# joncampbell123/composite-video-simulator

Measured on AMD Instinct MI355X. Metric: frames/sec (output frames = fields; 720x486 NTSC, preset '-vhs'; steady-state pipelined throughput, 4 steps in flight), higher is better.
Workload: dtype f64; 1 GPU; 720x486 30fps 10s colour-bars clip, preset '-vhs': 300 frames -> 600 fields per GPU per step, frame-round-robin over 1 GPU(s); steps_in_flight=4, mode=exact (bit-identical to the reference: fp64, no FMA contraction)

## Files before the change

### composite-video-simulator_amd/csrc/ntsc_decode_fast.hip

```cpp
#pragma clang fp contract(off)

namespace ntscsim {
namespace fastdec {

typedef uint32_t v4u __attribute__((ext_vector_type(4)));
#ifdef NTSC_PLAIN_OUT_STORES
#define NTSC_OUT_STORE(p, v) (*(p) = (v))
#else
#define NTSC_OUT_STORE(p, v) __builtin_nontemporal_store((v), (p))
#endif
typedef __attribute__((address_space(1))) v4u *g_v4u_ptr;
typedef __attribute__((address_space(1))) const v4u *g_cv4u_ptr;
DEV v4u to_v4u(const uint4 &a) { return v4u{a.x, a.y, a.z, a.w}; }
typedef __attribute__((address_space(1))) uint32_t *g_u32_ptr;
typedef __attribute__((address_space(1))) const uint32_t *g_cu32_ptr;

#ifdef NTSC_NO_STEP_SCHED_BARRIER
#define NTSC_STEP_SCHED_BARRIER() ((void)0)
#else
#define NTSC_STEP_SCHED_BARRIER() __builtin_amdgcn_sched_barrier(0)
#endif

struct LaneRand32 {
    uint32_t p3, p2, p1;
    int pos;
    DEV void init(uint32_t *ring, const uint32_t *state, int stride, int lane, int o)
    {
        for (int j = 0; j < 31; j++) {
            const uint32_t w = state[(size_t)j * stride];
            const int sl = (o + j) & 31;
            ring[sl * 64 + lane] = w;
            if (sl == 0) ring[32 * 64 + lane] = w;
            if (j == 28) p3 = w;
            if (j == 29) p2 = w;
            if (j == 30) p1 = w;
        }
        pos = (o + 31) & 31;
    }
    DEV uint32_t next(uint32_t *ring, int lane)
    {
        const uint32_t v = ring[(pos + 1) * 64 + lane] + p3;
        ring[pos * 64 + lane] = v;
        if (pos == 0) ring[32 * 64 + lane] = v;
        p3 = p2; p2 = p1; p1 = v;
        pos = (pos + 1) & 31;
        return v >> 1;
    }
    template <int K>
    DEV uint32_t draw(uint32_t *rb, bool first_slot_is_zero)
    {
        const uint32_t v = rb[(K + 1) * 64] + p3;
        rb[K * 64] = v;
        if (K == 0 && first_slot_is_zero) rb[32 * 64] = v;
        p3 = p2; p2 = p1; p1 = v;
        return v >> 1;
    }
};

template <class RT>
struct Casc3;
template <>
struct Casc3<double> {
    double r0, r1, r2;
    DEV void reset(double v, double a) { const double r = v - (v * a); r0 = r1 = r2 = r; }
    DEV double push(double s, double a, double &m2)
    {
        const double p0 = (s * a) + r0;
        const double m0 = p0 * a;
        r0 = p0 - m0;
// ... 153 lines not shown
            if (ANY) {
                const int aL = odd ? o2 : e2, aH = odd ? o1 : e1;
                const int bL = odd ? e1 : o2, bH = odd ? ch : o1;
                a = hi ? aH : aL; b = hi ? bH : bL;
                const int sg = NEG ? ~mo : mo;
                a = (a ^ sg) - sg; b = (b ^ sg) - sg;
            } else {
                a = hi ? e1 : e2; b = hi ? o1 : o2;
                if (NEG) { a = -a; b = -b; }
            }
            e2 = e1; e1 = ch;
            if (MASK) { a &= dm; b &= dm; }
            ieN = a; qeN = b;
            Io = (ieP + ieN) >> 1;
            Qo = (qeP + qeN) >> 1;
        } else {
            o2 = o1; o1 = ch;
            Io = ieN; Qo = qeN;
            ieP = ieN; qeP = qeN;
        }
    }
};

template <bool VHS, class RT>
struct State {
    DemodR D1, D2;
    int l0, l1, l2, lsum;
    Casc3<RT> vl, vcU, vcV, sh, oU, oV;
    PoleHp<RT> vpre;
    int Yprev, Uraw, Vraw;
    RT Uf2[2];
    LaneRand32 rng;
    int nU, nV;
};

template <class RT, bool WR = false, bool BK = false, bool SV = false, bool XA = false, bool FO = false>
struct Const {
    static constexpr bool fullout = FO;
    static constexpr int SH = FO ? 3 : 0;
    RT a_oi, a_oq;
    uint32_t *xs;
    static constexpr bool wraps = WR;
    static constexpr bool back = BK;
    static constexpr bool svideo = SV;
    static constexpr bool anyxi = XA;
    bool odd;
    int mo;
    int ms[4];
    unsigned bmul, bshift;
    int wrapoff;
    int wrapA, wrapS;
    unsigned xi;
    bool hi;
    int W, xe, lane;
    int d, SKT, LOFF;
    int mL, mNL;
    int bA, bC;
    int dm;
    RT cosv, sinv;
    RT a_vc, a_vl, a_sh, a_tv, sharp2;
    int *tailU;
    size_t rstride;
    __amdgpu_buffer_rsrc_t comp;
    int vbase;
    int rowbytes;
};
// ... 94 lines not shown
{
    int Y, U, V;
    constexpr bool pick3 = ((J + 1 + CT::SH) & 1) != 0;
    constexpr bool neg3 = ((J + 1 + CT::SH) & 3) == 3;
    if constexpr (!VHS) {
        T.D1.template push<pick3, neg3, true, CT::back, true, CT::anyxi>(pc, C.hi, C.dm, Y, U, V, C.bmul, C.bshift, C.odd, C.mo);
    } else {
        int Yv, Uv, Vv;
        const int c2 = vcr_step<DPH, J, RT, CT>(P, S, T, C, pc, pl, Yv, Uv, Vv);
        if constexpr (CT::svideo) {
            Y = Yv; U = Uv & C.dm; V = Vv & C.dm;
        } else {
            T.D2.template push<pick3, neg3, true, false, true, CT::anyxi>(c2, C.hi, C.dm, Y, U, V, 0, 0, C.odd, C.mo);
        }
    }
    if constexpr (CT::fullout) {
        const int fUn = (int)S.oU.push((RT)U, C.a_oi);
        const RT fVd = rtrunc<RT>(S.oV.push((RT)V, C.a_oq));
        const int Yo = T.yd[J];
        T.yd[J] = Y;
        const RT fUd = (RT)T.ud[J & 1];
        T.ud[J & 1] = fUn;
        return yiq_to_bgra<RT>(Yo, fUd, fVd);
    } else {
        const RT fUd = rtrunc<RT>(S.oU.push((RT)U, C.a_tv));
        const RT fVd = rtrunc<RT>(S.oV.push((RT)V, C.a_tv));
        const int Yo = S.Yprev;
        S.Yprev = Y;
        return yiq_to_bgra<RT>(Yo, fUd, fVd);
    }
}

template <class RT, class CT>
DEV int vcr_edge(const DevParams &P, State<true, RT> &S, const CT &C, uint32_t *ring, int t, int &Yv, int &Uv, int &Vv)
{
    const int W = C.W;
    const int pc = t < W ? cs_load(C, t) : 0;
    int Y, U, V;
    S.D1.template push_edge<CT::back, CT::anyxi>(pc, t, C.xi, C.hi, W, C.xe, Y, U, V, C.bmul, C.bshift);
    const int x1 = t - 7;
    const bool in1 = x1 >= 0 && x1 < W;
    int fU = 0, fV = 0;
    if (in1) {
        U += S.nU; V += S.nV;
        S.nU = sdiv2(S.nU + (int)umod31(S.rng.next(ring, C.lane), P.m_cnoise) - P.cnoise_k);
        S.nV = sdiv2(S.nV + (int)umod31(S.rng.next(ring, C.lane), P.m_cnoise) - P.cnoise_k);
        const RT u = (RT)U, v = (RT)V;
        U = (int)((u * C.cosv) - (v * C.sinv));
        V = (int)((u * C.sinv) + (v * C.cosv));
        fU = (int)S.vcU.push((RT)U, C.a_vc);
        fV = (int)S.vcV.push((RT)V, C.a_vc);
        if (x1 >= W - C.d) {
            C.tailU[(size_t)(x1 & 15) * C.rstride] = U;
            C.tailU[(size_t)(16 + (x1 & 15)) * C.rstride] = V;
        }
    }
    const int x2 = x1 - C.d;
    const int xl = t - C.LOFF;
    const int pl = (xl >= 0 && xl < W) ? cs_load(C, xl) : 0;
    const int yb = sdiv4(S.l0 + S.l1 + S.l2 + pl);
    S.lsum = S.l1 + S.l2 + pl;
    S.l0 = S.l1; S.l1 = S.l2; S.l2 = pl;
    const bool in2 = x2 >= 0 && x2 < W;
    if (in2) {
        if (x2 >= W - C.d) {
            fU = C.tailU[(size_t)(x2 & 15) * C.rstride];
            fV = C.tailU[(size_t)(16 + (x2 & 15)) * C.rstride];
        }
        RT m2;
        RT s = S.vl.push((RT)yb, C.a_vl, m2);
        s += S.vpre.hp(s, m2, C.a_vl) * RT(1.6);
        const RT s0 = rtrunc<RT>(s);
        const RT ts = S.sh.push(s0, C.a_sh);
        Y = (int)(s0 + ((s0 - ts) * C.sharp2));
    }
    U = ((wave_up(fU) & C.bA) + fU + C.bC) >> C.bC;
    V = ((wave_up(fV) & C.bA) + fV + C.bC) >> C.bC;
    int c2 = 0;
    Yv = 0; Uv = 0; Vv = 0;
    if (in2) {
        Yv = Y; Uv = U; Vv = V;
        const unsigned s = (C.xi + (unsigned)x2) & 3u;
        int chroma = (s & 1u) ? V : U;
        if (s & 2u) chroma = -chroma;
        c2 = Y + chroma;
    }
    return c2;
}

template <bool VHS, class RT, class CT>
DEV bool edge_step(const DevParams &P, State<VHS, RT> &S, const CT &C, uint32_t *ring, int t,
                   uint32_t &px, int &xo_out)
{
    const int W = C.W;
    int Y, U, V;
    int x3 = t - 7;
    if constexpr (VHS) {
        int Yv, Uv, Vv;
        const int c2 = vcr_edge<RT, CT>(P, S, C, ring, t, Yv, Uv, Vv);
        const int x2 = t - 7 - C.d;
        if constexpr (CT::svideo) {
            Y = Yv; U = Uv; V = Vv;
            x3 = x2;
        } else {
            S.D2.template push_edge<false, CT::anyxi>(c2, x2, C.xi, C.hi, W, C.xe, Y, U, V);
            x3 = x2 - 7;
        }
    } else {
        const int pc = t < W ? cs_load(C, t) : 0;
        S.D1.template push_edge<CT::back, CT::anyxi>(pc, t, C.xi, C.hi, W, C.xe, Y, U, V, C.bmul, C.bshift);
    }
    if constexpr (CT::fullout) {
        if (x3 < 0 || x3 >= W + 4) return false;
        const bool in3f = x3 < W;
        if (!in3f) { U = 0; V = 0; Y = 0; }
        U &= C.dm; V &= C.dm;
        RT fUn = 0, fVn = 0;
        if (in3f) {
            fUn = rtrunc<RT>(S.oU.push((RT)U, C.a_oi));
            fVn = rtrunc<RT>(S.oV.push((RT)V, C.a_oq));
        }
        const int k3 = x3 & 3;
        const int Yo4 = (int)C.xs[k3 * 64], Ur4 = (int)C.xs[(4 + k3) * 64], Vr4 = (int)C.xs[(8 + k3) * 64];
        C.xs[k3 * 64] = (uint32_t)Y; C.xs[(4 + k3) * 64] = (uint32_t)U; C.xs[(8 + k3) * 64] = (uint32_t)V;
        const RT Uf = S.Uf2[0];
        S.Uf2[0] = S.Uf2[1]; S.Uf2[1] = fUn;
        const int xof = x3 - 4;
        if (xof < 0) return false;
        const RT Uo = xof < W - 2 ? Uf : (RT)Ur4;
        const RT Vo = xof < W - 4 ? fVn : (RT)Vr4;
        px = yiq_to_bgra<RT>(Yo4, Uo, Vo);
        xo_out = xof;
        return true;
    }
    if (x3 < 0 || x3 > W) return false;
    const bool in3 = x3 < W;
    if (!in3) { U = 0; V = 0; Y = 0; }
    U &= C.dm; V &= C.dm;
    RT fUd = 0, fVd = 0;
    if (in3) {
        fUd = rtrunc<RT>(S.oU.push((RT)U, C.a_tv));
        fVd = rtrunc<RT>(S.oV.push((RT)V, C.a_tv));
    }
    const int xo = x3 - 1;
    const int Yo = S.Yprev;
    const int Ur = S.Uraw, Vr = S.Vraw;
    S.Yprev = Y; S.Uraw = U; S.Vraw = V;
    if (xo < 0) return false;
    if (xo >= W - 1) { fUd = (RT)Ur; fVd = (RT)Vr; }
    px = yiq_to_bgra<RT>(Yo, fUd, fVd);
    xo_out = xo;
    return true;
}

template <bool VHS, int DPH, class RT, class CT>
DEV int steady(const DevParams &P, State<VHS, RT> &S, const CT &C, uint32_t *ring, uint32_t *lring,
               uint32_t *ostage, const unsigned long long *orow, uint32_t *drow, bool is_out, int t)
{
    const int t_end = C.W - (C.d > 7 ? C.d - 7 : 0);
    const int SKT = C.SKT, LOFF = C.LOFF, lane = C.lane;
    if (t + 4 > t_end) return t;
    if (VHS && (S.rng.pos & 7)) return t;
    Steady T;
    constexpr bool pick3_next = ((1 + CT::SH) & 1) != 0;
    T.D1.from(S.D1, VHS ? (DPH & 1) != 0 : pick3_next);
    T.D2.from(S.D2, pick3_next);
    T.lc1 = S.l2; T.lpA = S.l2 + S.l1; T.lpB = S.l1 + S.l0;
    if constexpr (CT::fullout) {
#pragma unroll
        for (int q = 0; q < 4; q++) T.yd[q] = (int)C.xs[q * 64];
        T.ud[0] = (int)S.Uf2[0]; T.ud[1] = (int)S.Uf2[1];
    }
    DemodS &Dout = (VHS && !CT::svideo) ? T.D2 : T.D1;
    if (!(VHS && CT::svideo)) { Dout.ieP &= C.dm; Dout.qeP &= C.dm; Dout.ieN &= C.dm; Dout.qeN &= C.dm; }
    int sbase = VHS ? S.rng.pos : 0;
    constexpr int PD = 4;
    int pc[PD], pl[PD];
#pragma unroll
    for (int j = 0; j < PD; j++) { pc[j] = cs_load(C, t + j); pl[j] = VHS ? cs_load<NTSC_COMP_LOAD2_AUX>(C, t + j - LOFF) : 0; }
    constexpr bool PFTOP = !VHS;
    int pend_x = -1;
#ifdef NTSC_FAST_LANE_STORE
#define NTSC_FAST_FLUSH()                                                                         \
    if (pend_x >= 0) {                                                                            \
        if (is_out) {                                                                             \
// ... 66 lines not shown
#pragma unroll
        for (int q = 0; q < 4; q++) C.xs[q * 64] = (uint32_t)T.yd[q];
        S.Uf2[0] = (RT)T.ud[0]; S.Uf2[1] = (RT)T.ud[1];
    }
    S.Uraw = 0; S.Vraw = 0;
    S.l2 = T.lc1; S.l1 = T.lpA - T.lc1; S.l0 = T.lpB - S.l1; S.lsum = S.l0 + S.l1 + S.l2;
    if (VHS) S.rng.pos = sbase;
    return t;
}

}

#ifndef NTSC_FAST_WAVES
#define NTSC_FAST_WAVES 2
#endif
#ifndef NTSC_FAST_WAVES_F32
#define NTSC_FAST_WAVES_F32 2
#endif
template <class RT> struct FastWaves { static constexpr int n = NTSC_FAST_WAVES; };
template <> struct FastWaves<float> { static constexpr int n = NTSC_FAST_WAVES_F32; };
template <bool VHS, class RT, bool WR, bool BK, bool SV = false, bool XA = false, bool FO = false>
DEV void decode_fast_body(const DevParams &P, const GeomDev &G, const FieldDev *__restrict__ fields,
                          const int *__restrict__ comp, const uint32_t *__restrict__ rs_chroma,
                          const int *__restrict__ n0_u, const int *__restrict__ n0_v,
                          const int *__restrict__ hs_shift, const int *__restrict__ pn_noise,
                          const int *__restrict__ dropout, int *__restrict__ tails)
{
    using namespace fastdec;
    __shared__ uint32_t ring[33 * 64];
    __shared__ uint32_t lring[FO ? 12 * 64 : 64];
    __shared__ __attribute__((aligned(16))) uint32_t ostage[64 * 20];
    __shared__ unsigned long long orow[64];

    const int lane = threadIdx.x;
    const int gidx = blockIdx.x * 63 + lane - 1;
    const int rc = gidx < 0 ? 0 : (gidx < P.R ? gidx : P.R - 1);
    const int f = rc / P.Lslot, k = rc - f * P.Lslot;
    const FieldDev &fd = fields[f];
    const unsigned field = fd.field & 1u;
    const bool rowok = (int)(field + 2u * k) < P.H;
#ifdef NTSC_AB_NOSTORE
    const bool is_out = false;
#else
    const bool is_out = lane >= 1 && gidx < P.R && rowok;
#endif
    const unsigned y = rowok ? field + 2u * (unsigned)k : field;
    const int W = P.W;
    uint32_t *drow = reinterpret_cast<uint32_t *>(fd.dst + (size_t)fd.dst_ls * y);
    orow[lane] = is_out ? (unsigned long long)drow : 0ull;
    const size_t tcol = (size_t)blockIdx.x * 64 + lane;
    const size_t tstride = (size_t)gridDim.x * 64;

    typedef Const<RT, WR, BK, SV, XA, FO> CT;
    CT C;
    C.bmul = P.m_amp_back.mul; C.bshift = P.m_amp_back.shift;
    C.xi = scan_phase(P, y, fd.fieldno);
    C.hi = (C.xi & 2u) != 0;
    C.odd = (C.xi & 1u) != 0;
    if constexpr (XA) {
        C.mo = opaque_v(C.odd ? -1 : 0);
#pragma unroll
        for (int j = 0; j < 4; j++) C.ms[j] = opaque_v(((C.xi + (unsigned)j) & 2u) ? -1 : 0);
    }
    C.W = W;
    C.xe = (W & 1) ? W - 1 : W - 2;
    C.lane = lane;
    C.d = VHS ? P.cdelay : 0;
    C.SKT = (VHS ? (CT::svideo ? 8 : 15) + C.d : 8) + CT::SH;
    C.LOFF = 5 + C.d;
    C.mL = opaque_v(C.hi ? -1 : 0);
    C.mNL = opaque_v(~C.mL);
    const bool vb = VHS && P.vblend && P.ntsc;
    C.bA = opaque_v((vb && k >= 2) ? -1 : 0);
    C.bC = opaque_v((vb && k >= 1) ? 1 : 0);
    C.dm = opaque_v((P.loss && dropout[rc] != 0) ? 0 : -1);
    C.cosv = 1; C.sinv = 0;
    if (VHS) {
        int n = (rowok ? pn_noise[rc] : 0) + P.pnoise_k;
        n = n < 0 ? 0 : (n > 2 * P.pnoise_k ? 2 * P.pnoise_k : n);
        C.cosv = (RT)G.ptab[2 * n]; C.sinv = (RT)G.ptab[2 * n + 1];
    }
    C.a_vc = (RT)P.a_vc; C.a_vl = (RT)P.a_vl; C.a_sh = (RT)P.a_sh; C.a_tv = (RT)P.a_tv;
    C.a_oi = (RT)P.a_in_i; C.a_oq = (RT)P.a_in_q;
    C.sharp2 = (RT)(P.sharpen * 2);
    C.tailU = tails + tcol;
    C.rstride = tstride;
    C.rowbytes = P.Rpad * 4;
    const int hs = P.hs ? hs_shift[rc] : 0;
    C.vbase = (int)((unsigned)rc * 4u + (unsigned)hs * (unsigned)C.rowbytes);
    {
        const int tw = W + W / 10;
        C.wrapoff = (int)((unsigned)(hs > 0 ? -tw : tw) * (unsigned)C.rowbytes);
        C.wrapA = hs > 0 ? tw - hs - 1 : (hs < 0 ? -hs - 1 : 0x3FFFFFFF);
        C.wrapS = opaque_v(hs < 0 ? -1 : 0);
    }
    C.comp = __builtin_amdgcn_make_buffer_rsrc(const_cast<int *>(comp), 0,
                                               (int)((unsigned)W * (unsigned)C.rowbytes), 0x00020000);

    State<VHS, RT> S;
    S.D1.init(); S.D2.init();
    S.l0 = S.l1 = S.l2 = S.lsum = 0;
    S.vl.reset(16, C.a_vl); S.vpre.reset(16, C.a_vl); S.vcU.reset(0, C.a_vc); S.vcV.reset(0, C.a_vc);
    S.sh.reset(0, C.a_sh);
    if (CT::fullout) { S.oU.reset(0, C.a_oi); S.oV.reset(0, C.a_oq); }
    else { S.oU.reset(0, C.a_tv); S.oV.reset(0, C.a_tv); }
    S.Yprev = S.Uraw = S.Vraw = 0;
    C.xs = lring + lane;
    if (CT::fullout)
        for (int q = 0; q < 12; q++) C.xs[q * 64] = 0;
    S.Uf2[0] = S.Uf2[1] = 0;
    S.nU = S.nV = 0;
    if (VHS) {
        const int fill_draws = 2 * (C.SKT - 7);
        S.rng.init(ring, rs_chroma + rc, P.Rpad, lane, (-(31 + fill_draws)) & 7);
        S.nU = n0_u[rc]; S.nV = n0_v[rc];
    }

    const int SKT = C.SKT;
    const int total = W + SKT;
    int t = 0;
#ifdef NTSC_EDGE_UNROLL
#pragma unroll NTSC_EDGE_UNROLL
#endif
    for (; t < SKT && t < total; t++) {
        uint32_t px; int xo;
        (void)edge_step<VHS, RT, CT>(P, S, C, ring, t, px, xo);
    }
    if constexpr (!VHS) t = steady<VHS, 0, RT, CT>(P, S, C, ring, lring, ostage, orow, drow, is_out, t);
    else switch ((C.SKT - 7) & 3) {
        case 0: t = steady<VHS, 0, RT, CT>(P, S, C, ring, lring, ostage, orow, drow, is_out, t); break;
        case 1: t = steady<VHS, 1, RT, CT>(P, S, C, ring, lring, ostage, orow, drow, is_out, t); break;
        case 2: t = steady<VHS, 2, RT, CT>(P, S, C, ring, lring, ostage, orow, drow, is_out, t); break;
        default: t = steady<VHS, 3, RT, CT>(P, S, C, ring, lring, ostage, orow, drow, is_out, t); break;
    }
#ifdef NTSC_EDGE_UNROLL
#pragma unroll NTSC_EDGE_UNROLL
#endif
    for (; t < total; t++) {
        uint32_t px; int xo;
        if (!edge_step<VHS, RT, CT>(P, S, C, ring, t, px, xo)) continue;
        ostage[lane * 20 + (xo & 15)] = px;
        if ((xo & 15) == 15) {
            if (is_out) {
                const uint4 *sp = reinterpret_cast<const uint4 *>(&ostage[lane * 20]);
                g_v4u_ptr dp = (g_v4u_ptr)(drow + (xo - 15));
                const uint4 a = sp[0], b = sp[1], c4 = sp[2], d4 = sp[3];
                dp[0] = to_v4u(a); dp[1] = to_v4u(b); dp[2] = to_v4u(c4); dp[3] = to_v4u(d4);
            }
        } else if (xo == W - 1 && is_out) {
            const int xb = xo & ~15;
            for (int q = xb; q <= xo; q++) ((g_u32_ptr)drow)[q] = ostage[lane * 20 + (q - xb)];
        }
    }
}

template <bool VHS, class RT, bool WR = false>
__global__ __launch_bounds__(64, VHS ? FastWaves<RT>::n : 4) void k_decode_fast(DevParams P, GeomDev G,
                                                     const FieldDev *__restrict__ fields,
                                                     const int *__restrict__ comp,
                                                     const uint32_t *__restrict__ rs_chroma,
                                                     const int *__restrict__ n0_u,
                                                     const int *__restrict__ n0_v,
                                                     const int *__restrict__ hs_shift,
                                                     const int *__restrict__ pn_noise,
                                                     const int *__restrict__ dropout,
                                                     int *__restrict__ tails)
{
    decode_fast_body<VHS, RT, WR, false>(P, G, fields, comp, rs_chroma, n0_u, n0_v, hs_shift, pn_noise, dropout, tails);
}

template <bool VHS, class RT>
__global__ __launch_bounds__(64, VHS ? FastWaves<RT>::n : 4) void k_decode_fast_bk(DevParams P, GeomDev G,
                                                     const FieldDev *__restrict__ fields,
                                                     const int *__restrict__ comp,
                                                     const uint32_t *__restrict__ rs_chroma,
                                                     const int *__restrict__ n0_u,
                                                     const int *__restrict__ n0_v,
                                                     const int *__restrict__ hs_shift,
                                                     const int *__restrict__ pn_noise,
                                                     const int *__restrict__ dropout,
                                                     int *__restrict__ tails)
{
    decode_fast_body<VHS, RT, VHS, true>(P, G, fields, comp, rs_chroma, n0_u, n0_v, hs_shift, pn_noise, dropout, tails);
}

template <class RT>
// ... 82 lines not shown
    C.d = P.cdelay;
    C.SKT = 7 + C.d;
    C.LOFF = 5 + C.d;
    C.mL = opaque_v(C.hi ? -1 : 0);
    C.mNL = opaque_v(~C.mL);
    const bool vb = P.vblend && P.ntsc;
    C.bA = opaque_v((vb && k >= 2) ? -1 : 0);
    C.bC = opaque_v((vb && k >= 1) ? 1 : 0);
    C.dm = -1;
    {
        int n = (rowok ? pn_noise[rc] : 0) + P.pnoise_k;
        n = n < 0 ? 0 : (n > 2 * P.pnoise_k ? 2 * P.pnoise_k : n);
        C.cosv = (RT)G.ptab[2 * n]; C.sinv = (RT)G.ptab[2 * n + 1];
    }
    C.a_vc = (RT)P.a_vc; C.a_vl = (RT)P.a_vl; C.a_sh = (RT)P.a_sh; C.a_tv = (RT)P.a_tv;
    C.sharp2 = (RT)(P.sharpen * 2);
    C.tailU = tails + tcol;
    C.rstride = tstride;
    C.rowbytes = P.Rpad * 4;
    const int hs = P.hs ? hs_shift[rc] : 0;
    C.vbase = (int)((unsigned)rc * 4u + (unsigned)hs * (unsigned)C.rowbytes);
    C.comp = __builtin_amdgcn_make_buffer_rsrc(const_cast<int *>(comp), 0,
                                               (int)((unsigned)W * (unsigned)C.rowbytes), 0x00020000);
    const __amdgpu_buffer_rsrc_t out = __builtin_amdgcn_make_buffer_rsrc(comp_out, 0,
                                               (int)((unsigned)W * (unsigned)C.rowbytes), 0x00020000);
    const int vout = (is_out ? gidx : P.R + lane) * 4;

    State<true, RT> S;
    S.D1.init(); S.D2.init();
    S.l0 = S.l1 = S.l2 = S.lsum = 0;
    S.vl.reset(16, C.a_vl); S.vpre.reset(16, C.a_vl); S.vcU.reset(0, C.a_vc); S.vcV.reset(0, C.a_vc);
    S.sh.reset(0, C.a_sh); S.oU.reset(0, C.a_tv); S.oV.reset(0, C.a_tv);
    S.Yprev = S.Uraw = S.Vraw = 0;
    S.rng.init(ring, rs_chroma + rc, P.Rpad, lane, (-(31 + 2 * (C.SKT - 7))) & 7);
    S.nU = n0_u[rc]; S.nV = n0_v[rc];

    const int SK1 = C.SKT, LOFF = C.LOFF;
    const int total = W + SK1;
    const unsigned rb = (unsigned)C.rowbytes;
    int t = 0;
    int yv_, uv_, vv_;
    for (; t < SK1 && t < total; t++) (void)vcr_edge<RT, CT>(P, S, C, ring, t, yv_, uv_, vv_);
    {
        const int t_end = W - (C.d > 7 ? C.d - 7 : 0);
        if (t + 4 <= t_end && !(S.rng.pos & 7)) {
            Steady T;
            T.D1.from(S.D1, (C.d & 1) != 0);
            T.D2.from(S.D2, true);
            T.lc1 = S.l2; T.lpA = S.l2 + S.l1; T.lpB = S.l1 + S.l0;
            int sbase = S.rng.pos;
            int pc[4], pl[4];
#pragma unroll
            for (int j = 0; j < 4; j++) { pc[j] = cs_load(C, t + j); pl[j] = cs_load<NTSC_COMP_LOAD2_AUX>(C, t + j - LOFF); }
            unsigned soff = (unsigned)(t - SK1) * rb;
#define NTSC_VCR_STEP(DPV, J)                                                                     \
            {                                                                                     \
                const int c2 = vcr_step<DPV, J, RT, CT>(P, S, T, C, pc[J], pl[J], yv_, uv_, vv_); \
                pc[J] = cs_load(C, t + 4 + J);         \
                pl[J] = cs_load<NTSC_COMP_LOAD2_AUX>(C, t + 4 + J - LOFF);                                             \
                __builtin_amdgcn_raw_buffer_store_b32(c2, out, vout, (int)soff, 0);               \
                soff += rb;                                                                       \
                NTSC_STEP_SCHED_BARRIER();                                                        \
            }
#define NTSC_VCR_ITER(DPV)                                                                        \
            for (; t + 4 <= t_end; t += 4) {                                                      \
                T.rb = ring + sbase * 64 + lane; T.rb0 = sbase == 0; sbase = (sbase + 8) & 31;    \
                NTSC_VCR_STEP(DPV, 0) NTSC_VCR_STEP(DPV, 1) NTSC_VCR_STEP(DPV, 2) NTSC_VCR_STEP(DPV, 3)  \
            }
            switch (C.d & 3) {
                case 0: NTSC_VCR_ITER(0) break;
                case 1: NTSC_VCR_ITER(1) break;
                case 2: NTSC_VCR_ITER(2) break;
                default: NTSC_VCR_ITER(3) break;
            }
#undef NTSC_VCR_ITER
#undef NTSC_VCR_STEP
            T.D1.to(S.D1, (C.d & 1) != 0);
            S.l2 = T.lc1; S.l1 = T.lpA - T.lc1; S.l0 = T.lpB - S.l1; S.lsum = S.l0 + S.l1 + S.l2;
            S.rng.pos = sbase;
        }
    }
    for (; t < total; t++) {
        const int c2 = vcr_edge<RT, CT>(P, S, C, ring, t, yv_, uv_, vv_);
        const int x2 = t - SK1;
        if (x2 >= 0) __builtin_amdgcn_raw_buffer_store_b32(c2, out, vout, (int)((unsigned)x2 * rb), 0);
    }
}

}
```

### composite-video-simulator_amd/csrc/ntsc_encode_fast.hip

```cpp
#pragma clang fp contract(off)

#ifndef NTSC_COMP_STORE_AUX
#define NTSC_COMP_STORE_AUX 2
#endif
#ifdef NTSC_ENC_LOAD_NT
#define NTSC_ENC_LOAD(p) __builtin_nontemporal_load(p)
#else
#define NTSC_ENC_LOAD(p) (*(p))
#endif
namespace ntscsim {
namespace fastenc {

using fastdec::Casc3;
using fastdec::opaque_v;

template <class RT>
struct EState {
    Casc3<RT> lpI, lpQ;
    int Yd[4];
    int Ir[4], Qr[4];
    int fI[2];
    fastdec::LaneRand32 rng;
    int noise;
    OnePoleT<RT> pre;
// ... 144 lines not shown
#pragma unroll
        for (int i = 0; i < 4; i++) {
            const int from = 16 * i + (lane >> 2);
            const unsigned l2 = (unsigned)__shfl((int)lo, from), h2 = (unsigned)__shfl((int)hi, from);
            ptr[i] = (const uint8_t *)(((uintptr_t)h2 << 32) | l2) + 16 * (lane & 3);
        }
        wr = (lane >> 2) * 20 + (lane & 3) * 4;
        rd = lane * 20;
    }
    DEV void request(int t0, fastdec::v4u (&q)[4]) const
    {
#pragma unroll
        for (int i = 0; i < 4; i++) q[i] = NTSC_ENC_LOAD((fastdec::g_cv4u_ptr)(ptr[i] + 4 * (size_t)t0));
    }
    DEV void deliver(const fastdec::v4u (&q)[4], uint32_t (&px)[16]) const
    {
#pragma unroll
        for (int i = 0; i < 4; i++) *reinterpret_cast<uint4 *>(&tile[16 * 20 * i + wr]) = make_uint4(q[i].x, q[i].y, q[i].z, q[i].w);
#pragma unroll
        for (int i = 0; i < 4; i++) {
            const uint4 v = *reinterpret_cast<const uint4 *>(&tile[rd + 4 * i]);
            px[4 * i] = v.x; px[4 * i + 1] = v.y; px[4 * i + 2] = v.z; px[4 * i + 3] = v.w;
        }
    }
};

}

template <class RT, bool PRE, bool XA = false, int GH = 0>
DEV void encode_fast_body(const DevParams &P, const FieldDev *__restrict__ fields, const uint32_t *__restrict__ rs_luma,
                          const int *__restrict__ n0_luma, int *__restrict__ comp)
{
    using namespace fastenc;
    __shared__ uint32_t ring[33 * 64];
#ifndef NTSC_ENC_NOCOOP
    __shared__ __attribute__((aligned(16))) uint32_t ltile[64 * 20];
#endif
    __shared__ uint32_t gring[GH ? NTSC_GHOST_RING * 64 : 1];
    const int lane = threadIdx.x;
    const int rho = blockIdx.x * 64 + lane;
    const int rc = rho < P.R ? rho : P.R - 1;
    const int f = rc / P.Lslot, k = rc - f * P.Lslot;
    const FieldDev &fd = fields[f];
    const unsigned field = fd.field & 1u;
    const bool valid = rho < P.R && (int)(field + 2u * k) < P.H;
    const unsigned y = valid ? field + 2u * (unsigned)k : field;
    const unsigned opposite = (fd.flags & 1u) ? ((fd.flags & 2u) ? 1u : 0u) : 0u;
    unsigned sy = y + opposite;
    if (sy > (unsigned)P.H - 1u) sy = (unsigned)P.H - 1u;
    const uint8_t *srow = fd.src + (size_t)fd.src_ls * sy;
    const int W = P.W;

    EConst<RT> C;
    C.xi = scan_phase(P, y, fd.fieldno);
    C.W = W;
    C.lane = lane;
    C.mL = opaque_v((C.xi & 2u) ? -1 : 0);
    C.mNL = opaque_v(~C.mL);
    C.odd = (C.xi & 1u) != 0;
#pragma unroll
    for (int j = 0; j < 4; j++) C.ms[j] = fastdec::opaque_v(((C.xi + (unsigned)j) & 2u) ? -1 : 0);
    C.a_i = (RT)P.a_in_i; C.a_q = (RT)P.a_in_q;
    C.a_pre = (RT)P.a_pre; C.pre_gain = (RT)P.pre_gain;
    C.rowbytes = P.Rpad * 4;
    C.vcol = rho * 4;
    C.comp = __builtin_amdgcn_make_buffer_rsrc(comp, 0, (int)((unsigned)W * (unsigned)C.rowbytes), 0x00020000);

    EState<RT> S;
    S.rng.init(ring, rs_luma + rc, P.Rpad, lane, 1);
    S.noise = n0_luma[rc];
    S.lpI.reset(0, C.a_i); S.lpQ.reset(0, C.a_q);
    S.pre.p = 16;
#pragma unroll
    for (int q = 0; q < 4; q++) { S.Yd[q] = 0; S.Ir[q] = 0; S.Qr[q] = 0; }
    S.fI[0] = S.fI[1] = 0;
    GhostRing<GH> gh;
    gh.begin(P, gring, lane);

    int t = 0;
    for (; t < 4; t++) edge_step<RT, PRE, GH>(P, S, C, ring, reinterpret_cast<const uint32_t *>(srow), t, gh);
    if (t + 16 <= W) {
#ifndef NTSC_ENC_NOCOOP
        CoopLoader L;
        L.begin(srow, ltile, lane);
        uint32_t cur[16];
        fastdec::v4u nq[4];
        L.request(t, nq);
        L.deliver(nq, cur);
#else
        uint32_t cur[16], nxt[16];
        load_chunk(srow, t, cur);
#endif
        int Y0 = S.Yd[0], Y1 = S.Yd[1], Y2 = S.Yd[2], Y3 = S.Yd[3];
        int I0 = S.fI[0], I1 = S.fI[1];
        RT IdT[4], QdT[4];
        int sbase = S.rng.pos;
        for (; t + 16 <= W; t += 16) {
            const bool more = t + 32 <= W;
            uint32_t *const rb = ring + sbase * 64 + lane;
            const bool rb0 = sbase == 0;
            sbase = (sbase + 16) & 31;
#ifndef NTSC_ENC_NOCOOP
            if (more) L.request(t + 16, nq);
#else
            if (more) load_chunk(srow, t + 16, nxt);
#endif
            unsigned soff = (unsigned)(t - 4) * (unsigned)C.rowbytes;
            int Yn[16], F[16];
#define NTSC_ENC_STEP(J, YX, IX)                                                                  \
            {                                                                                     \
                RT dY, Id_, Qd_;                                                                  \
                rgb_to_yiq256<RT>(cur[J], dY, Id_, Qd_);                                          \
                Yn[J] = (int)dY;                                                                  \
// ... 6 lines not shown
            NTSC_ENC_STEP(1, Y1, I1)
            NTSC_ENC_STEP(2, Y2, F[0])
            NTSC_ENC_STEP(3, Y3, F[1])
            NTSC_ENC_STEP(4, Yn[0], F[2])
            NTSC_ENC_STEP(5, Yn[1], F[3])
            NTSC_ENC_STEP(6, Yn[2], F[4])
            NTSC_ENC_STEP(7, Yn[3], F[5])
            NTSC_ENC_STEP(8, Yn[4], F[6])
            NTSC_ENC_STEP(9, Yn[5], F[7])
            NTSC_ENC_STEP(10, Yn[6], F[8])
            NTSC_ENC_STEP(11, Yn[7], F[9])
            NTSC_ENC_STEP(12, Yn[8], F[10])
            NTSC_ENC_STEP(13, Yn[9], F[11])
            NTSC_ENC_STEP(14, Yn[10], F[12])
            NTSC_ENC_STEP(15, Yn[11], F[13])
#undef NTSC_ENC_STEP
            Y0 = Yn[12]; Y1 = Yn[13]; Y2 = Yn[14]; Y3 = Yn[15];
            I0 = F[14]; I1 = F[15];
#ifndef NTSC_ENC_NOCOOP
            if (more) L.deliver(nq, cur);
#else
            if (more) {
#pragma unroll
                for (int j = 0; j < 16; j++) cur[j] = nxt[j];
            }
#endif
        }
        S.rng.pos = sbase;
        S.Yd[0] = Y0; S.Yd[1] = Y1; S.Yd[2] = Y2; S.Yd[3] = Y3;
        S.fI[0] = I0; S.fI[1] = I1;
#pragma unroll
        for (int q = 0; q < 4; q++) { S.Ir[q] = (int)IdT[q]; S.Qr[q] = (int)QdT[q]; }
    }
    for (; t < W + 4; t++) edge_step<RT, PRE, GH>(P, S, C, ring, reinterpret_cast<const uint32_t *>(srow), t, gh);
}

template <class RT>
__global__ __launch_bounds__(64) void k_encode_fast(DevParams P, const FieldDev *__restrict__ fields,
                                                    const uint32_t *__restrict__ rs_luma,
                                                    const int *__restrict__ n0_luma,
                                                    int *__restrict__ comp)
{
    encode_fast_body<RT, false>(P, fields, rs_luma, n0_luma, comp);
}

template <class RT, int GT>
__global__ __launch_bounds__(64) void k_encode_fast_gh(DevParams P, const FieldDev *__restrict__ fields,
                                                       const uint32_t *__restrict__ rs_luma,
                                                       const int *__restrict__ n0_luma,
                                                       int *__restrict__ comp)
{
    encode_fast_body<RT, false, false, GT>(P, fields, rs_luma, n0_luma, comp);
}

template <class RT>
__global__ __launch_bounds__(64) void k_encode_fast_xi(DevParams P, const FieldDev *__restrict__ fields,
                                                       const uint32_t *__restrict__ rs_luma,
                                                       const int *__restrict__ n0_luma,
                                                       int *__restrict__ comp)
{
    encode_fast_body<RT, false, true>(P, fields, rs_luma, n0_luma, comp);
}

template <class RT>
__global__ __launch_bounds__(64) void k_encode_fast_pre(DevParams P, const FieldDev *__restrict__ fields,
                                                        const uint32_t *__restrict__ rs_luma,
                                                        const int *__restrict__ n0_luma,
// ... 7 lines not shown
```

### composite-video-simulator_amd/csrc/ntscsim_hip.hip

```cpp
#include <hip/hip_runtime.h>

#include <algorithm>
#include <cmath>
#include <cstdio>
#include <cstdlib>
#include <cstring>
#include <mutex>
#include <unistd.h>
#include <new>
#include <string>
#include <vector>

#include "ntscsim.h"
#include "ntsc_device.hpp"

#include "ntsc_kernels.hip"
#include "ntsc_decode_fast.hip"
#include "ntsc_encode_fast.hip"
#include "ntsc_pipe.hip"
#include "ntsc422_kernels.hip"
#include "ntsc422_fused.hip"
#include "ntsc_scale.hip"
#include "ntsc_float.hpp"
#include "ntsc_blend.hpp"
// ... 486 lines not shown
        c->ev_free.push_back(s);
        n++;
    }
    c->ev_live.clear();
    if (n_calls) *n_calls = n;
    return NTSCSIM_OK;
}

extern "C" int ntscsim_set_mode(ntscsim_ctx *c, int mode)
{
    if (!c || (mode != NTSCSIM_MODE_EXACT && mode != NTSCSIM_MODE_FAST32 && mode != NTSCSIM_MODE_FLOAT)) return NTSCSIM_E_ARG;
    c->mode = mode;
    return NTSCSIM_OK;
}

extern "C" void ntscsim_debug_force_generic(ntscsim_ctx *c, int on)
{
    if (c) c->force_generic = on != 0;
}

extern "C" void ntscsim_debug_no_fast_decode(ntscsim_ctx *c, int on)
{
    if (c) { c->no_fast_decode = (on & 1) != 0; c->split_vhs = (on & 2) != 0; c->no_stream422 = (on & 4) != 0; c->no_ghost_fuse = (on & 8) != 0; c->no_setup_merge = (on & 16) != 0; }
}

extern "C" int ntscsim_debug_last_kernels(const ntscsim_ctx *c, char *out, size_t cap)
{
    if (!c || !out || cap == 0) return NTSCSIM_E_ARG;
    const size_t n = std::min(cap - 1, c->kernels.size());
    std::memcpy(out, c->kernels.data(), n);
    out[n] = 0;
    return (int)c->kernels.size();
}

extern "C" void ntscsim_debug_set_warmup(ntscsim_ctx *c, int luma_draws, int chroma_draws)
{
    if (!c) return;
    c->warm_override[0] = luma_draws;
    c->warm_override[1] = chroma_draws & ~1;
    (void)hipSetDevice(c->device);
    (void)hipDeviceSynchronize();
    for (Geometry *e : c->geoms) e->valid = false;
}

#ifndef NTSC_SETUP_MERGE_MAX
#define NTSC_SETUP_MERGE_MAX 64
#endif
static void launch_setup_kernels(ntscsim_ctx *c, const DevParams &D, const GeomDev &G, const FieldDev *fields_dev, int n, hipStream_t st,
                                 bool note, bool launch)
{
    const bool fs = D.hs || D.pnoise_k || D.loss, rs = D.noise_k || D.cnoise_k;
    if (fs && rs && n <= NTSC_SETUP_MERGE_MAX && !c->no_setup_merge) {
        const int nfs = 3 * n, nrs = (D.R + 63) / 64;
        if (note) note_kernel(c, "k_field_row_setup");
        if (launch)
        hipLaunchKernelGGL(k_field_row_setup, dim3((unsigned)(nfs + 2 * nrs)), dim3(64), 0, st, D, G, fields_dev,
                           c->hs_shift.p, c->pn_noise.p, c->dropout.p, c->rs_luma.p, c->n0_luma.p, c->rs_chroma.p,
                           c->n0_u.p, c->n0_v.p, nfs, nrs);
        return;
    }
    if (fs) {
        if (note) note_kernel(c, "k_field_setup");
        if (launch)
        hipLaunchKernelGGL(k_field_setup, dim3((n + 63) / 64), dim3(64), 0, st, D, G, fields_dev,
                           c->hs_shift.p, c->pn_noise.p, c->dropout.p);
    }
// ... 1501 lines not shown
```

Measured before the change: 805,800 frames/s.

## Prefetch edge samples ahead in decode edge loops and hoist per-row loads

Moves the composite sample loads out of the per-step edge function and issues them four steps ahead in a new edge_run loop, masking out-of-range values afterwards. The tail chroma read is prefetched one step early into state registers, and per-row side inputs (dropout, phase noise, h-shift, initial noise, RNG ring) are loaded at kernel entry. The RNG init is unrolled into batched loads. This is meant to hide global-memory latency in the serial head and tail phases, at the cost of extra registers and clamped redundant loads. Optional cycle-stamp probes are added behind a compile flag.

```diff
diff --git a/composite-video-simulator_amd/csrc/ntsc_decode_fast.hip b/composite-video-simulator_amd/csrc/ntsc_decode_fast.hip
--- a/composite-video-simulator_amd/csrc/ntsc_decode_fast.hip
+++ b/composite-video-simulator_amd/csrc/ntsc_decode_fast.hip
@@ -1,6 +1,24 @@
 #pragma clang fp contract(off)
 
 namespace ntscsim {
+#ifdef NTSC_PHASE_STAMPS
+__device__ unsigned long long g_phase_cycles[2][8];
+#define NTSC_PHASE_STAMP(v) const unsigned long long v = (unsigned long long)__builtin_readcyclecounter()
+DEV void phase_add(int which, int lane, unsigned long long t0, unsigned long long t1, unsigned long long t2,
+                   unsigned long long t3, unsigned long long t4)
+{
+    if (lane != 0) return;
+    atomicAdd(&g_phase_cycles[which][0], t1 - t0);
+    atomicAdd(&g_phase_cycles[which][1], t2 - t1);
+    atomicAdd(&g_phase_cycles[which][2], t3 - t2);
+    atomicAdd(&g_phase_cycles[which][3], t4 - t3);
+    atomicAdd(&g_phase_cycles[which][4], 1ull);
+}
+#define NTSC_PHASE_ADD(which, lane, t0, t1, t2, t3, t4) phase_add(which, lane, t0, t1, t2, t3, t4)
+#else
+#define NTSC_PHASE_STAMP(v) ((void)0)
+#define NTSC_PHASE_ADD(which, lane, t0, t1, t2, t3, t4) ((void)0)
+#endif
 namespace fastdec {
 
 typedef uint32_t v4u __attribute__((ext_vector_type(4)));
@@ -26,15 +44,13 @@
     int pos;
     DEV void init(uint32_t *ring, const uint32_t *state, int stride, int lane, int o)
     {
-        for (int j = 0; j < 31; j++) {
-            const uint32_t w = state[(size_t)j * stride];
-            const int sl = (o + j) & 31;
-            ring[sl * 64 + lane] = w;
-            if (sl == 0) ring[32 * 64 + lane] = w;
-            if (j == 28) p3 = w;
-            if (j == 29) p2 = w;
-            if (j == 30) p1 = w;
-        }
+        uint32_t w[31];
+#pragma unroll
+        for (int j = 0; j < 31; j++) w[j] = state[(size_t)j * stride];
+#pragma unroll
+        for (int j = 0; j < 31; j++) ring[((o + j) & 31) * 64 + lane] = w[j];
+        ring[32 * 64 + lane] = ring[lane];
+        p3 = w[28]; p2 = w[29]; p1 = w[30];
         pos = (o + 31) & 31;
     }
     DEV uint32_t next(uint32_t *ring, int lane)
@@ -254,6 +270,7 @@
     RT Uf2[2];
     LaneRand32 rng;
     int nU, nV;
+    int tU, tV;
 };
 
 template <class RT, bool WR = false, bool BK = false, bool SV = false, bool XA = false, bool FO = false>
@@ -414,10 +431,10 @@
 }
 
 template <class RT, class CT>
-DEV int vcr_edge(const DevParams &P, State<true, RT> &S, const CT &C, uint32_t *ring, int t, int &Yv, int &Uv, int &Vv)
+DEV int vcr_edge(const DevParams &P, State<true, RT> &S, const CT &C, uint32_t *ring, int t, int pc, int pl,
+                 int &Yv, int &Uv, int &Vv)
 {
     const int W = C.W;
-    const int pc = t < W ? cs_load(C, t) : 0;
     int Y, U, V;
     S.D1.template push_edge<CT::back, CT::anyxi>(pc, t, C.xi, C.hi, W, C.xe, Y, U, V, C.bmul, C.bshift);
     const int x1 = t - 7;
@@ -438,17 +455,12 @@
         }
     }
     const int x2 = x1 - C.d;
-    const int xl = t - C.LOFF;
-    const int pl = (xl >= 0 && xl < W) ? cs_load(C, xl) : 0;
     const int yb = sdiv4(S.l0 + S.l1 + S.l2 + pl);
     S.lsum = S.l1 + S.l2 + pl;
     S.l0 = S.l1; S.l1 = S.l2; S.l2 = pl;
     const bool in2 = x2 >= 0 && x2 < W;
     if (in2) {
-        if (x2 >= W - C.d) {
-            fU = C.tailU[(size_t)(x2 & 15) * C.rstride];
-            fV = C.tailU[(size_t)(16 + (x2 & 15)) * C.rstride];
-        }
+        if (x2 >= W - C.d) { fU = S.tU; fV = S.tV; }
         RT m2;
         RT s = S.vl.push((RT)yb, C.a_vl, m2);
         s += S.vpre.hp(s, m2, C.a_vl) * RT(1.6);
@@ -458,6 +470,11 @@
     }
     U = ((wave_up(fU) & C.bA) + fU + C.bC) >> C.bC;
     V = ((wave_up(fV) & C.bA) + fV + C.bC) >> C.bC;
+    const int x2n = x2 + 1;
+    if (x2n >= 0 && x2n < W && x2n >= W - C.d) {
+        S.tU = C.tailU[(size_t)(x2n & 15) * C.rstride];
+        S.tV = C.tailU[(size_t)(16 + (x2n & 15)) * C.rstride];
+    }
     int c2 = 0;
     Yv = 0; Uv = 0; Vv = 0;
     if (in2) {
@@ -471,7 +488,7 @@
 }
 
 template <bool VHS, class RT, class CT>
-DEV bool edge_step(const DevParams &P, State<VHS, RT> &S, const CT &C, uint32_t *ring, int t,
+DEV bool edge_step(const DevParams &P, State<VHS, RT> &S, const CT &C, uint32_t *ring, int t, int pc, int pl,
                    uint32_t &px, int &xo_out)
 {
     const int W = C.W;
@@ -479,7 +496,7 @@
     int x3 = t - 7;
     if constexpr (VHS) {
         int Yv, Uv, Vv;
-        const int c2 = vcr_edge<RT, CT>(P, S, C, ring, t, Yv, Uv, Vv);
+        const int c2 = vcr_edge<RT, CT>(P, S, C, ring, t, pc, pl, Yv, Uv, Vv);
         const int x2 = t - 7 - C.d;
         if constexpr (CT::svideo) {
             Y = Yv; U = Uv; V = Vv;
@@ -489,7 +506,6 @@
             x3 = x2 - 7;
         }
     } else {
-        const int pc = t < W ? cs_load(C, t) : 0;
         S.D1.template push_edge<CT::back, CT::anyxi>(pc, t, C.xi, C.hi, W, C.xe, Y, U, V, C.bmul, C.bshift);
     }
     if constexpr (CT::fullout) {
@@ -533,6 +549,66 @@
     px = yiq_to_bgra<RT>(Yo, fUd, fVd);
     xo_out = xo;
     return true;
+}
+
+template <bool VHS, class CT>
+DEV void edge_samples(const CT &C, int t, int &pc, int &pl)
+{
+    const int xl = t - C.LOFF;
+    pc = t < C.W ? cs_load(C, t) : 0;
+    pl = (VHS && xl >= 0 && xl < C.W) ? cs_load(C, xl) : 0;
+}
+template <bool VHS, class CT>
+DEV void edge_request(const CT &C, int t, int &pc, int &pl)
+{
+    const int wl = C.W - 1, xl = t - C.LOFF;
+    pc = cs_load(C, t < wl ? t : wl);
+    pl = VHS ? cs_load(C, xl < 0 ? 0 : (xl < wl ? xl : wl)) : 0;
+}
+template <class CT>
+DEV void edge_mask(const CT &C, int t, int &pc, int &pl)
+{
+    const int xl = t - C.LOFF;
+    pc &= opaque_s(t < C.W ? -1 : 0);
+    pl &= opaque_s((xl >= 0 && xl < C.W) ? -1 : 0);
+}
+
+template <bool VHS, bool EMIT, class RT, class CT>
+DEV int edge_run(const DevParams &P, State<VHS, RT> &S, const CT &C, uint32_t *ring, uint32_t *ostage, uint32_t *drow,
+                 bool is_out, int t, int tend)
+{
+    const int lane = C.lane, W = C.W;
+    int qc[4], ql[4];
+#pragma unroll
+    for (int j = 0; j < 4; j++) edge_request<VHS>(C, t + j, qc[j], ql[j]);
+    for (; t < tend; t += 4) {
+#pragma unroll
+        for (int j = 0; j < 4; j++) {
+            if (t + j < tend) {
+                int pc = qc[j], pl = ql[j];
+                edge_mask(C, t + j, pc, pl);
+                uint32_t px; int xo;
+                const bool have = edge_step<VHS, RT, CT>(P, S, C, ring, t + j, pc, pl, px, xo);
+                if (EMIT && have) {
+                    ostage[lane * 20 + (xo & 15)] = px;
+                    if ((xo & 15) == 15) {
+                        if (is_out) {
+                            const uint4 *sp = reinterpret_cast<const uint4 *>(&ostage[lane * 20]);
+                            g_v4u_ptr dp = (g_v4u_ptr)(drow + (xo - 15));
+                            const uint4 a = sp[0], b = sp[1], c4 = sp[2], d4 = sp[3];
+                            dp[0] = to_v4u(a); dp[1] = to_v4u(b); dp[2] = to_v4u(c4); dp[3] = to_v4u(d4);
+                        }
+                    } else if (xo == W - 1 && is_out) {
+                        const int xb = xo & ~15;
+                        for (int q = xb; q <= xo; q++) ((g_u32_ptr)drow)[q] = ostage[lane * 20 + (q - xb)];
+                    }
+                }
+            }
+            edge_request<VHS>(C, t + 4 + j, qc[j], ql[j]);
+            NTSC_STEP_SCHED_BARRIER();
+        }
+    }
+    return tend;
 }
 
 template <bool VHS, int DPH, class RT, class CT>
@@ -665,11 +741,22 @@
     __shared__ __attribute__((aligned(16))) uint32_t ostage[64 * 20];
     __shared__ unsigned long long orow[64];
 
+    NTSC_PHASE_STAMP(ph0);
     const int lane = threadIdx.x;
     const int gidx = blockIdx.x * 63 + lane - 1;
     const int rc = gidx < 0 ? 0 : (gidx < P.R ? gidx : P.R - 1);
     const int f = rc / P.Lslot, k = rc - f * P.Lslot;
-    const FieldDev &fd = fields[f];
+    struct { decltype(FieldDev::field) field; decltype(FieldDev::fieldno) fieldno; decltype(FieldDev::dst) dst;
+             decltype(FieldDev::dst_ls) dst_ls; } fd = {fields[f].field, fields[f].fieldno, fields[f].dst, fields[f].dst_ls};
+    const int q_drop = *(P.loss ? dropout + rc : comp + rc);
+    const int q_pn = VHS ? pn_noise[rc] : 0;
+    const int q_hs = *(P.hs ? hs_shift + rc : comp + rc);
+    const int q_nu = VHS ? n0_u[rc] : 0, q_nv = VHS ? n0_v[rc] : 0;
+    State<VHS, RT> S;
+    {
+        const int skt = (VHS ? (SV ? 8 : 15) + P.cdelay : 8) + (FO ? 3 : 0);
+        if (VHS) S.rng.init(ring, rs_chroma + rc, P.Rpad, lane, (-(31 + 2 * (skt - 7))) & 7);
+    }
     const unsigned field = fd.field & 1u;
     const bool rowok = (int)(field + 2u * k) < P.H;
 #ifdef NTSC_AB_NOSTORE
@@ -706,10 +793,10 @@
     const bool vb = VHS && P.vblend && P.ntsc;
     C.bA = opaque_v((vb && k >= 2) ? -1 : 0);
     C.bC = opaque_v((vb && k >= 1) ? 1 : 0);
-    C.dm = opaque_v((P.loss && dropout[rc] != 0) ? 0 : -1);
+    C.dm = opaque_v((P.loss && q_drop != 0) ? 0 : -1);
     C.cosv = 1; C.sinv = 0;
     if (VHS) {
-        int n = (rowok ? pn_noise[rc] : 0) + P.pnoise_k;
+        int n = (rowok ? q_pn : 0) + P.pnoise_k;
         n = n < 0 ? 0 : (n > 2 * P.pnoise_k ? 2 * P.pnoise_k : n);
         C.cosv = (RT)G.ptab[2 * n]; C.sinv = (RT)G.ptab[2 * n + 1];
     }
@@ -719,7 +806,7 @@
     C.tailU = tails + tcol;
     C.rstride = tstride;
     C.rowbytes = P.Rpad * 4;
-    const int hs = P.hs ? hs_shift[rc] : 0;
+    const int hs = P.hs ? q_hs : 0;
     C.vbase = (int)((unsigned)rc * 4u + (unsigned)hs * (unsigned)C.rowbytes);
     {
         const int tw = W + W / 10;
@@ -730,7 +817,6 @@
     C.comp = __builtin_amdgcn_make_buffer_rsrc(const_cast<int *>(comp), 0,
                                                (int)((unsigned)W * (unsigned)C.rowbytes), 0x00020000);
 
-    State<VHS, RT> S;
     S.D1.init(); S.D2.init();
     S.l0 = S.l1 = S.l2 = S.lsum = 0;
     S.vl.reset(16, C.a_vl); S.vpre.reset(16, C.a_vl); S.vcU.reset(0, C.a_vc); S.vcV.reset(0, C.a_vc);
@@ -742,23 +828,25 @@
     if (CT::fullout)
         for (int q = 0; q < 12; q++) C.xs[q * 64] = 0;
     S.Uf2[0] = S.Uf2[1] = 0;
-    S.nU = S.nV = 0;
-    if (VHS) {
-        const int fill_draws = 2 * (C.SKT - 7);
-        S.rng.init(ring, rs_chroma + rc, P.Rpad, lane, (-(31 + fill_draws)) & 7);
-        S.nU = n0_u[rc]; S.nV = n0_v[rc];
-    }
+    S.nU = q_nu; S.nV = q_nv;
+    S.tU = S.tV = 0;
 
     const int SKT = C.SKT;
     const int total = W + SKT;
     int t = 0;
+    NTSC_PHASE_STAMP(ph1);
+    constexpr bool AHEAD = !FO;
+    if constexpr (AHEAD) t = edge_run<VHS, false, RT, CT>(P, S, C, ring, ostage, drow, is_out, t, SKT);
+    else
 #ifdef NTSC_EDGE_UNROLL
 #pragma unroll NTSC_EDGE_UNROLL
 #endif
     for (; t < SKT && t < total; t++) {
-        uint32_t px; int xo;
-        (void)edge_step<VHS, RT, CT>(P, S, C, ring, t, px, xo);
-    }
+        uint32_t px; int xo, pc, pl;
+        edge_samples<VHS>(C, t, pc, pl);
+        (void)edge_step<VHS, RT, CT>(P, S, C, ring, t, pc, pl, px, xo);
+    }
+    NTSC_PHASE_STAMP(ph2);
     if constexpr (!VHS) t = steady<VHS, 0, RT, CT>(P, S, C, ring, lring, ostage, orow, drow, is_out, t);
     else switch ((C.SKT - 7) & 3) {
         case 0: t = steady<VHS, 0, RT, CT>(P, S, C, ring, lring, ostage, orow, drow, is_out, t); break;
@@ -766,12 +854,16 @@
         case 2: t = steady<VHS, 2, RT, CT>(P, S, C, ring, lring, ostage, orow, drow, is_out, t); break;
         default: t = steady<VHS, 3, RT, CT>(P, S, C, ring, lring, ostage, orow, drow, is_out, t); break;
     }
+    NTSC_PHASE_STAMP(ph3);
+    if constexpr (AHEAD) t = edge_run<VHS, true, RT, CT>(P, S, C, ring, ostage, drow, is_out, t, total);
+    else
 #ifdef NTSC_EDGE_UNROLL
 #pragma unroll NTSC_EDGE_UNROLL
 #endif
     for (; t < total; t++) {
-        uint32_t px; int xo;
-        if (!edge_step<VHS, RT, CT>(P, S, C, ring, t, px, xo)) continue;
+        uint32_t px; int xo, pc, pl;
+        edge_samples<VHS>(C, t, pc, pl);
+        if (!edge_step<VHS, RT, CT>(P, S, C, ring, t, pc, pl, px, xo)) continue;
         ostage[lane * 20 + (xo & 15)] = px;
         if ((xo & 15) == 15) {
             if (is_out) {
@@ -785,6 +877,8 @@
             for (int q = xb; q <= xo; q++) ((g_u32_ptr)drow)[q] = ostage[lane * 20 + (q - xb)];
         }
     }
+    NTSC_PHASE_STAMP(ph4);
+    NTSC_PHASE_ADD(0, lane, ph0, ph1, ph2, ph3, ph4);
 }
 
 template <bool VHS, class RT, bool WR = false>
@@ -933,6 +1027,7 @@
     S.vl.reset(16, C.a_vl); S.vpre.reset(16, C.a_vl); S.vcU.reset(0, C.a_vc); S.vcV.reset(0, C.a_vc);
     S.sh.reset(0, C.a_sh); S.oU.reset(0, C.a_tv); S.oV.reset(0, C.a_tv);
     S.Yprev = S.Uraw = S.Vraw = 0;
+    S.tU = S.tV = 0;
     S.rng.init(ring, rs_chroma + rc, P.Rpad, lane, (-(31 + 2 * (C.SKT - 7))) & 7);
     S.nU = n0_u[rc]; S.nV = n0_v[rc];
 
@@ -941,7 +1036,11 @@
     const unsigned rb = (unsigned)C.rowbytes;
     int t = 0;
     int yv_, uv_, vv_;
-    for (; t < SK1 && t < total; t++) (void)vcr_edge<RT, CT>(P, S, C, ring, t, yv_, uv_, vv_);
+    for (; t < SK1 && t < total; t++) {
+        int pc, pl;
+        edge_samples<true>(C, t, pc, pl);
+        (void)vcr_edge<RT, CT>(P, S, C, ring, t, pc, pl, yv_, uv_, vv_);
+    }
     {
         const int t_end = W - (C.d > 7 ? C.d - 7 : 0);
         if (t + 4 <= t_end && !(S.rng.pos & 7)) {
@@ -982,7 +1081,9 @@
         }
     }
     for (; t < total; t++) {
-        const int c2 = vcr_edge<RT, CT>(P, S, C, ring, t, yv_, uv_, vv_);
+        int pc, pl;
+        edge_samples<true>(C, t, pc, pl);
+        const int c2 = vcr_edge<RT, CT>(P, S, C, ring, t, pc, pl, yv_, uv_, vv_);
         const int x2 = t - SK1;
         if (x2 >= 0) __builtin_amdgcn_raw_buffer_store_b32(c2, out, vout, (int)((unsigned)x2 * rb), 0);
     }
diff --git a/composite-video-simulator_amd/csrc/ntsc_encode_fast.hip b/composite-video-simulator_amd/csrc/ntsc_encode_fast.hip
--- a/composite-video-simulator_amd/csrc/ntsc_encode_fast.hip
+++ b/composite-video-simulator_amd/csrc/ntsc_encode_fast.hip
@@ -200,6 +200,7 @@
                           const int *__restrict__ n0_luma, int *__restrict__ comp)
 {
     using namespace fastenc;
+    NTSC_PHASE_STAMP(ph0);
     __shared__ uint32_t ring[33 * 64];
 #ifndef NTSC_ENC_NOCOOP
     __shared__ __attribute__((aligned(16))) uint32_t ltile[64 * 20];
@@ -246,7 +247,9 @@
     gh.begin(P, gring, lane);
 
     int t = 0;
+    NTSC_PHASE_STAMP(ph1);
     for (; t < 4; t++) edge_step<RT, PRE, GH>(P, S, C, ring, reinterpret_cast<const uint32_t *>(srow), t, gh);
+    NTSC_PHASE_STAMP(ph2);
     if (t + 16 <= W) {
 #ifndef NTSC_ENC_NOCOOP
         CoopLoader L;
@@ -319,7 +322,10 @@
 #pragma unroll
         for (int q = 0; q < 4; q++) { S.Ir[q] = (int)IdT[q]; S.Qr[q] = (int)QdT[q]; }
     }
+    NTSC_PHASE_STAMP(ph3);
     for (; t < W + 4; t++) edge_step<RT, PRE, GH>(P, S, C, ring, reinterpret_cast<const uint32_t *>(srow), t, gh);
+    NTSC_PHASE_STAMP(ph4);
+    NTSC_PHASE_ADD(1, lane, ph0, ph1, ph2, ph3, ph4);
 }
 
 template <class RT>
diff --git a/composite-video-simulator_amd/csrc/ntscsim_hip.hip b/composite-video-simulator_amd/csrc/ntscsim_hip.hip
--- a/composite-video-simulator_amd/csrc/ntscsim_hip.hip
+++ b/composite-video-simulator_amd/csrc/ntscsim_hip.hip
@@ -542,6 +542,20 @@
     out[n] = 0;
     return (int)c->kernels.size();
 }
+
+#ifdef NTSC_PHASE_STAMPS
+extern "C" int ntscsim_debug_phase_cycles(unsigned long long *out, int reset)
+{
+    if (!out) return NTSCSIM_E_ARG;
+    if (hipDeviceSynchronize() != hipSuccess) return NTSCSIM_E_HIP;
+    if (hipMemcpyFromSymbol(out, HIP_SYMBOL(g_phase_cycles), sizeof(g_phase_cycles)) != hipSuccess) return NTSCSIM_E_HIP;
+    if (reset) {
+        const unsigned long long zero[2][8] = {};
+        if (hipMemcpyToSymbol(HIP_SYMBOL(g_phase_cycles), zero, sizeof(zero)) != hipSuccess) return NTSCSIM_E_HIP;
+    }
+    return NTSCSIM_OK;
+}
+#endif
 
 extern "C" void ntscsim_debug_set_warmup(ntscsim_ctx *c, int luma_draws, int chroma_draws)
 {
```

After: 812,000 frames/s, median of 6. No clear change (+0.8%).
